# snf4j/snf4j

Measured on AMD Instinct MI355X. Metric: WebSocket frame decode GiB/s device-resident at 1/2/4/8 MI355X; % HBM peak, higher is better.
Workload: dtype u8; 1 GPU; 1048576 x 4096 B masked TEXT frames per GPU, 1024 sessions per GPU, unmask + UTF-8 validation, server-side decode (FrameDecoder+FrameUtf8Validator); frames_per_gpu=1048576, payload_bytes=4096, wire_bytes_per_gpu=4303355904, sessions_per_gpu=1024, parallelism=sessions sharded over 1 GPU(s), one process per GPU, no data-path collective

## Files before the change

snf4j_amd/build.py:

```python
from __future__ import annotations

import os
import subprocess
import sys
from concurrent.futures import ThreadPoolExecutor

HERE = os.path.dirname(os.path.abspath(__file__))
CSRC = os.path.join(HERE, "csrc")
OUT = os.path.join(HERE, "libwsgpu.so")
SOURCES = ["decode.hip", "encode.hip", "aggregate.hip", "api.hip", "batcher.hip", "inflate.hip", "handshake.hip", "deflate.hip"]
HEADERS = ["ws_rules.h", "wsgpu_internal.h", "wsgpu_scan.h", "deflate_core.h", "deflate_pmd.h", "../../include/wsgpu.h"]
BENCH_DIR = os.path.join(os.path.dirname(HERE), "benchsupport")
BENCH_SRC = os.path.join(BENCH_DIR, "csrc", "synth.hip")
BENCH_OUT = os.path.join(BENCH_DIR, "libwsbench.so")
BENCH_HDR = os.path.join(os.path.dirname(HERE), "include", "wsbench.h")
HIPCC = os.environ.get("HIPCC", "/opt/rocm/bin/hipcc")
FLAGS = ["--offload-arch=gfx950", "-O3", "-std=c++17", "-fPIC", "-Wall", "-Wno-unused-function",
         "-mllvm", "-disable-promote-alloca-to-lds"]


def _digest(paths, flags) -> str:
    import hashlib
    h = hashlib.sha256(" ".join(flags).encode())
    for p in paths:
        h.update(os.path.basename(p).encode())
        with open(p, "rb") as fh:
            h.update(fh.read())
    return h.hexdigest()


def _fresh(out: str, digest: str) -> bool:
    try:
        with open(out + ".srchash") as fh:
            return os.path.exists(out) and fh.read().strip() == digest
# ... 55 lines not shown
```

snf4j_amd/csrc/api.hip:

```cpp
#include <stdarg.h>
#include <stdio.h>
#include <stdlib.h>
#include <string.h>

#include <algorithm>
#include <atomic>
#include <string>
#include <vector>

#include "wsgpu_internal.h"

using namespace ws;

namespace {

std::atomic<uint64_t> g_ctx_allocs{0};

const char* const kKernelNames[K_COUNT] = {"k_parse",   "k_scan",     "k_link",     "k_piecesN",
                                           "k_final",    "k_enc_len",  "k_enc_scan",
                                           "k_enc_piecesN", "k_enc_final", "k_enc_desc", "k_agg_plan", "k_agg_gather", "k_inflate", "k_hs_accept", "k_infl_tok", "k_infl_fast", "k_hs_validate",
                                           "k_defl_plan", "k_defl_prep", "k_defl_match", "k_defl_parse", "k_defl_final", "k_defl_serial",
                                           "k_defl_trees", "k_defl_emit", "k_defl_hist", "k_defl_match_lds", "k_defl_links",
                                           "k_hs_accept_neg", "k_hs_validate_neg"};

// ... 295 lines not shown
}

int wsg_get_timing(wsg_ctx* c, double* out_ms, uint64_t* out_count, int max_kernels) {
  if (!c) return WSG_API_EINVAL;
  drain_timing(c);
  for (int i = 0; i < K_COUNT && i < max_kernels; ++i) {
    if (out_ms) out_ms[i] = c->ms[i];
    if (out_count) out_count[i] = c->count[i];
  }
  return K_COUNT;
}

int wsg_reset_timing(wsg_ctx* c) {
  if (!c) return WSG_API_EINVAL;
  drain_timing(c);
  memset(c->ms, 0, sizeof c->ms);
  memset(c->count, 0, sizeof c->count);
  return WSG_API_OK;
}

static int ensure_decode_ws(wsg_ctx* c, uint64_t n_frames, uint32_t n_sessions, uint64_t wire_len) {
  const uint64_t F = n_frames ? n_frames : 1;
  const uint64_t nblk = (F + DBLOCK - 1) / DBLOCK;
  HIP_TRY(c, c->pieces.ensure((piece_bound(wire_len, F) + 8) * sizeof(PieceDesc)));
  HIP_TRY(c, c->rec.ensure(F * sizeof(FrameRec)));
  HIP_TRY(c, c->vflag.ensure(F));
  HIP_TRY(c, c->slink.ensure(3 * (uint64_t)(n_sessions ? n_sessions : 1) * sizeof(int32_t)));
  HIP_TRY(c, c->edge.ensure(2 * F * sizeof(uint32_t)));
  HIP_TRY(c, c->blk_sum.ensure(nblk * sizeof(uint64_t)));
  HIP_TRY(c, c->blk_max.ensure(4 * ((nblk + 3) & ~3ull) * sizeof(int32_t)));
  HIP_TRY(c, c->chunk.ensure((nblk / SCAN_CHUNK + 1) * (sizeof(uint64_t) + 4 * sizeof(int32_t))));
  HIP_TRY(c, c->sess_err.ensure((uint64_t)(n_sessions ? n_sessions : 1) * sizeof(uint64_t), 0xff, c->stream));
  HIP_TRY(c, c->total.ensure(sizeof(uint64_t)));
  return WSG_API_OK;
}

static int ensure_encode_ws(wsg_ctx* c, uint64_t n_frames) {
  const uint64_t F = n_frames ? n_frames : 1;
  const uint64_t nblk = (F + BLOCK - 1) / BLOCK;
  HIP_TRY(c, c->esess.ensure(F * sizeof(uint32_t)));
  HIP_TRY(c, c->elast_close.ensure(F * sizeof(int32_t)));
  HIP_TRY(c, c->blk_sum.ensure(nblk * sizeof(uint64_t)));
  HIP_TRY(c, c->blk_max.ensure(3 * nblk * sizeof(int32_t)));
  return WSG_API_OK;
}

static constexpr uint64_t INFL_RESIDENT_LANES = 65536;
// ... 65 lines not shown
}
}

extern "C" {

int wsg_reserve(wsg_ctx* c, uint64_t max_frames, uint32_t max_sessions, uint64_t max_wire_len) {
  if (!c) return WSG_API_EINVAL;
  HIP_TRY(c, hipSetDevice(c->device));
  int rc = ensure_decode_ws(c, max_frames, max_sessions, max_wire_len);
  if (rc) return rc;
  return ensure_encode_ws(c, max_frames);
}

uint64_t wsg_decode_payload_bound(uint64_t wire_len, uint64_t n_frames) { return wire_len + 16 * n_frames + 16; }


int wsg_decode_batch_device(wsg_ctx* c, const wsg_decoder_cfg* cfg, const uint8_t* wire, uint64_t wire_len,
                            const uint64_t* frame_off, uint64_t n_frames, const uint32_t* session_first,
                            uint32_t n_sessions, wsg_session_state* state, uint8_t* payload_out,
                            uint64_t payload_cap, wsg_frame_desc* desc_out, wsg_session_result* result_out) {
  if (!c || !cfg) return WSG_API_EINVAL;
  if (n_sessions == 0) return n_frames ? set_err(c, WSG_API_EINVAL, "frames without sessions") : WSG_API_OK;
  if (n_frames >= (1ull << 30)) return set_err(c, WSG_API_ERANGE, "too many frames in one batch (max 2^30 - 1)");
  if (((uintptr_t)wire & 3) || ((uintptr_t)payload_out & 15))
    return set_err(c, WSG_API_EINVAL, "wire must be 4-B aligned and payload_out 16-B aligned");
  if (payload_cap < wire_len + 16 * n_frames)
    return set_err(c, WSG_API_ERANGE, "payload_cap below wsg_decode_payload_bound()");
  HIP_TRY(c, hipSetDevice(c->device));
  int rc = ensure_decode_ws(c, n_frames, n_sessions, wire_len);
  if (rc) return rc;
  DecodeArgs a;
  a.wire = wire;
  a.wire_len = wire_len;
  a.frame_off = frame_off;
  a.n_frames = n_frames;
  a.session_first = session_first;
  a.n_sessions = n_sessions;
  a.client_mode = cfg->client_mode != 0;
  a.allow_ext = cfg->allow_extensions != 0;
  a.validate = cfg->validate_utf8 != 0;
  a.max_payload = cfg->max_payload_len;
  a.state = state;
  a.payload_out = payload_out;
  a.desc = desc_out;
  a.result = result_out;
  a.rec = (FrameRec*)c->rec.p;
  a.vflag = (uint8_t*)c->vflag.p;
  a.slink = (int32_t*)c->slink.p;
  a.edge = (uint32_t*)c->edge.p;
  a.blk_sum = (uint64_t*)c->blk_sum.p;
  a.blk_max = (int32_t*)c->blk_max.p;
  a.chunk_sum = (uint64_t*)c->chunk.p;
  a.chunk_max = (int32_t*)(a.chunk_sum + (n_frames + DBLOCK - 1) / DBLOCK / SCAN_CHUNK + 1);
  a.sess_err = (uint64_t*)c->sess_err.p;
  a.total = (uint64_t*)c->total.p;
  a.pieces = (PieceDesc*)c->pieces.p;
  a.nblk = (uint32_t)((n_frames + DBLOCK - 1) / DBLOCK);
  a.n_pieces = piece_bound(wire_len, n_frames);
  a.validator_only = 0;
  a.in_desc = nullptr;
  a.sparse = (cfg->flags & WSG_CFG_SPARSE) != 0;
  a.fused_scan = a.nblk <= FUSED_SCAN_MAX_BLOCKS && c->fused_scan;
  if (n_frames) {
    timed(c, K_PARSE, [&] { launch_parse(a, c->stream); });
    if (!a.fused_scan) timed(c, K_SCAN, [&] { launch_scan(a, c->stream); });
    timed(c, K_LINK, [&] { launch_link(a, c->stream); });
    timed(c, K_UNMASK, [&] { launch_pieces(a, c->stream, piece_bound(wire_len, n_frames)); });
  }
  timed(c, K_FINAL, [&] { launch_final(a, c->stream); });
  HIP_TRY(c, hipGetLastError());
  return WSG_API_OK;
}

int wsg_validate_batch_device(wsg_ctx* c, const wsg_frame_desc* desc, uint64_t n_frames,
                              const uint32_t* session_first, uint32_t n_sessions, const uint8_t* payload,
                              uint64_t payload_len, wsg_session_state* state, wsg_session_result* result_out) {
  if (!c) return WSG_API_EINVAL;
  if (n_sessions == 0) return n_frames ? set_err(c, WSG_API_EINVAL, "frames without sessions") : WSG_API_OK;
  if (n_frames >= (1ull << 30)) return set_err(c, WSG_API_ERANGE, "too many frames in one batch (max 2^30 - 1)");
  if ((uintptr_t)payload & 3) return set_err(c, WSG_API_EINVAL, "payload must be 4-B aligned");
  HIP_TRY(c, hipSetDevice(c->device));
  int rc = ensure_decode_ws(c, n_frames, n_sessions, payload_len);
  if (rc) return rc;
  HIP_TRY(c, c->v_desc.ensure((n_frames + 1) * sizeof(wsg_frame_desc)));
  DecodeArgs a;
  a.wire = payload;
  a.wire_len = payload_len;
  a.frame_off = nullptr;
  a.n_frames = n_frames;
  a.session_first = session_first;
  a.n_sessions = n_sessions;
  a.client_mode = 0;
  a.allow_ext = 1;
  a.validate = 1;
  a.max_payload = INT64_MAX;
  a.state = state;
  a.payload_out = nullptr;
  a.desc = (wsg_frame_desc*)c->v_desc.p;
  a.result = result_out;
  a.rec = (FrameRec*)c->rec.p;
  a.vflag = (uint8_t*)c->vflag.p;
  a.slink = (int32_t*)c->slink.p;
  a.edge = (uint32_t*)c->edge.p;
  a.blk_sum = (uint64_t*)c->blk_sum.p;
  a.blk_max = (int32_t*)c->blk_max.p;
  a.chunk_sum = (uint64_t*)c->chunk.p;
  a.chunk_max = (int32_t*)(a.chunk_sum + (n_frames + DBLOCK - 1) / DBLOCK / SCAN_CHUNK + 1);
  a.sess_err = (uint64_t*)c->sess_err.p;
  a.total = (uint64_t*)c->total.p;
  a.pieces = (PieceDesc*)c->pieces.p;
  a.nblk = (uint32_t)((n_frames + DBLOCK - 1) / DBLOCK);
  a.n_pieces = piece_bound(payload_len, n_frames);
  a.validator_only = 1;
  a.in_desc = desc;
  a.sparse = 0;
  a.fused_scan = a.nblk <= FUSED_SCAN_MAX_BLOCKS && c->fused_scan;
  if (n_frames) {
    timed(c, K_PARSE, [&] { launch_vparse(a, c->stream); });
    if (!a.fused_scan) timed(c, K_SCAN, [&] { launch_scan(a, c->stream); });
    timed(c, K_LINK, [&] { launch_link(a, c->stream); });
    timed(c, K_UNMASK, [&] { launch_vpieces(a, c->stream, a.n_pieces); });
  }
  timed(c, K_FINAL, [&] { launch_final(a, c->stream); });
  HIP_TRY(c, hipGetLastError());
  return WSG_API_OK;
}

int wsg_validate_batch_host(wsg_ctx* c, const wsg_frame_desc* desc, uint64_t n_frames, const uint32_t* session_first,
                            uint32_t n_sessions, const uint8_t* payload, uint64_t payload_len, wsg_session_state* state,
                            wsg_session_result* result_out) {
  if (!c) return WSG_API_EINVAL;
  HIP_TRY(c, hipSetDevice(c->device));
  const uint64_t S = n_sessions;
  HIP_TRY(c, c->h_desc.ensure((n_frames + 1) * sizeof(wsg_frame_desc)));
  HIP_TRY(c, c->h_sf.ensure((S + 1) * sizeof(uint32_t)));
// ... 987 lines not shown
```

snf4j_amd/csrc/decode.hip:

```cpp
#include "wsgpu_internal.h"
#include "wsgpu_scan.h"

namespace ws {

__device__ bool utf8_valid_run(const uint8_t* wire, uint64_t off, uint32_t n, uint32_t mask, uint32_t phase0) {
  uint32_t p1 = 0, p2 = 0, p3 = 0;
  for (uint32_t i = 0; i < n; ++i) {
    uint32_t b = wire[off + i] ^ ((mask >> (8 * ((phase0 + i) & 3))) & 0xffu);
    if (utf8_err_byte(p3, p2, p1, b)) return false;
    p3 = p2; p2 = p1; p1 = b;
  }
  return !utf8_incomplete(p3, p2, p1);
}

struct DAgg {
  uint64_t sum;
  int32_t m0, m1, m2;
  uint32_t c3;
};
constexpr DAgg DAGG_ID = {0ull, -1, -1, -1, 0u};
constexpr uint32_t C3_RESET = 1u << 26;
constexpr uint32_t C3_PENDING = 1u << 27;

__device__ __forceinline__ uint32_t carry_op(uint32_t x, uint32_t y) {
// ... 321 lines not shown
    ex = agg_op(ex, e[i]);
  }
  if (threadIdx.x == 0) store_chunk(a, blockIdx.x, tot);
}

__device__ bool seam_utf8_error(uint32_t c3, uint32_t f3, uint32_t len, bool fin) {
  const uint32_t nc = (c3 >> 24) & 3u, nh = len < 3 ? len : 3u, n = nc + nh;
  const uint64_t win = (uint64_t)((c3 & 0xffffffu) >> (24 - 8 * nc)) | ((uint64_t)f3 << (8 * nc));
  for (uint32_t i = nc; i < n; ++i) {
    const uint32_t p1 = i >= 1 ? (uint32_t)(win >> (8 * (i - 1))) & 0xffu : 0u;
    const uint32_t p2 = i >= 2 ? (uint32_t)(win >> (8 * (i - 2))) & 0xffu : 0u;
    const uint32_t p3 = i >= 3 ? (uint32_t)(win >> (8 * (i - 3))) & 0xffu : 0u;
    if (utf8_err_byte(p3, p2, p1, (uint32_t)(win >> (8 * i)) & 0xffu)) return true;
  }
  if (fin && len < 3) {
    const uint32_t t1 = n >= 1 ? (uint32_t)(win >> (8 * (n - 1))) & 0xffu : 0u;
    const uint32_t t2 = n >= 2 ? (uint32_t)(win >> (8 * (n - 2))) & 0xffu : 0u;
    const uint32_t t3 = n >= 3 ? (uint32_t)(win >> (8 * (n - 3))) & 0xffu : 0u;
    if (utf8_incomplete(t3, t2, t1)) return true;
  }
  return false;
}

__device__ __forceinline__ void write_pieces(const DecodeArgs& a, bool live, uint64_t k, const FrameRec& r,
                                             uint64_t ex_sum, bool validate, bool cont, int lane) {
  const uint64_t slot = live ? (uint64_t)((r.len + 15u) & ~15u) : 0ull;
  const uint64_t slot_end = ex_sum + slot;
  const uint32_t pc0 = (uint32_t)((ex_sum + PIECE - 1) / PIECE);
  const uint32_t cnt = slot ? (uint32_t)((slot_end + PIECE - 1) / PIECE) - pc0 : 0u;
  uint32_t cum = cnt;
  cum = wave_incl_sum_u32(cum);
  const uint32_t T = (uint32_t)__builtin_amdgcn_readlane((int)cum, 63);
  cum -= cnt;
  if (!T) return;
  const uint32_t fk = (uint32_t)k | (validate ? 0x80000000u : 0u) | ((live && (r.code & CODE_FIN)) ? 0x40000000u : 0u);
  for (uint32_t t = lane; t < ((T + 63u) & ~63u); t += 64) {
    int o = 0;
#pragma unroll
    for (int step = 32; step >= 1; step >>= 1)
      if ((uint32_t)__shfl((int)cum, o + step, 64) <= t) o += step;
    const uint32_t o_cum = (uint32_t)__shfl((int)cum, o, 64);
    const uint32_t o_pc0 = (uint32_t)__shfl((int)pc0, o, 64);
    const uint64_t o_out = ((uint64_t)(uint32_t)__shfl((int)(uint32_t)(ex_sum >> 32), o, 64) << 32) |
                           (uint32_t)__shfl((int)(uint32_t)ex_sum, o, 64);
    const uint64_t o_src = ((uint64_t)(uint32_t)__shfl((int)(uint32_t)(r.src >> 32), o, 64) << 32) |
                           (uint32_t)__shfl((int)(uint32_t)r.src, o, 64);
    const uint32_t o_len = (uint32_t)__shfl((int)r.len, o, 64);
    const uint32_t o_mask = (uint32_t)__shfl((int)r.mask, o, 64);
    const uint32_t o_fk = (uint32_t)__shfl((int)fk, o, 64);
    const bool o_cont = __shfl((int)cont, o, 64) != 0;
    if (t >= T) continue;
    const uint64_t pc = (uint64_t)o_pc0 + (t - o_cum);
    if (pc >= a.n_pieces) continue;
    const uint64_t ps = pc * PIECE;
    const uint64_t o_end = o_out + ((o_len + 15u) & ~15u);
    const uint32_t j0 = (uint32_t)(ps - o_out);
    const uint32_t left = o_len - j0;
    const bool single = o_end >= ps + PIECE || (uint64_t)(o_fk & 0x3fffffffu) + 1 == a.n_frames;
    PieceDesc d;
    d.info = ((o_src + j0) & PD_SRC_MASK) | ((uint64_t)(left < PIECE ? left : PIECE) << PD_NB_SHIFT) |
             ((o_fk & 0x80000000u) ? PD_VALIDATE : 0ull) | (j0 == 0 ? PD_FIRST : 0ull) | (single ? 0ull : PD_MULTI) |
             (left <= PIECE ? PD_LAST : 0ull) | ((o_fk & 0x40000000u) ? PD_FIN : 0ull);
    d.mask = o_mask;
    d.frame = (o_fk & PDF_INDEX) | (o_cont ? PDF_CONT : 0u);
    a.pieces[pc] = d;
  }
}

__global__ __launch_bounds__(DBLOCK) void k_link(DecodeArgs a) {
  const int lane = threadIdx.x & 63;
  DAgg bp;
  if (a.fused_scan) {
    __shared__ uint32_t c3s[FUSED_SCAN_MAX_BLOCKS];
    DAgg t = DAGG_ID;
    const uint32_t nb = blockIdx.x, st = blk_stride(a);
    for (uint32_t b = threadIdx.x * 4u; b < nb; b += DBLOCK * 4u) {
      if (b + 4u <= nb) {
        const int4 x0 = *reinterpret_cast<const int4*>(a.blk_max + b);
        const int4 x1 = *reinterpret_cast<const int4*>(a.blk_max + st + b);
        const int4 x2 = *reinterpret_cast<const int4*>(a.blk_max + 2 * st + b);
        const int4 x3 = *reinterpret_cast<const int4*>(a.blk_max + 3 * st + b);
        const ulonglong2 s0 = *reinterpret_cast<const ulonglong2*>(a.blk_sum + b);
        const ulonglong2 s1 = *reinterpret_cast<const ulonglong2*>(a.blk_sum + b + 2);
        t.sum += s0.x + s0.y + s1.x + s1.y;
        t.m0 = max(max(t.m0, max(x0.x, x0.y)), max(x0.z, x0.w));
        t.m1 = max(max(t.m1, max(x1.x, x1.y)), max(x1.z, x1.w));
        t.m2 = max(max(t.m2, max(x2.x, x2.y)), max(x2.z, x2.w));
        c3s[b] = (uint32_t)x3.x;
// ... 59 lines not shown
        if (!a.validator_only) frag_err = rules_frag(op, frag);
        if (a.validate) {
          text = op == WSG_OP_TEXT;
          if (op == WSG_OP_CONTINUATION) text = jm >= sf ? (ex.m1 & 1) != 0 : (st.text_open != 0);
        }
      }
      uint32_t status = code_pre(r.code) ? code_pre(r.code) : (frag_err ? frag_err : code_post(r.code));
      if (!status && ex.sum + r.len > a.n_pieces * PIECE) status = WSG_E_BATCH;
      if (!status && text && op == WSG_OP_CONTINUATION &&
          seam_utf8_error(first ? tail_c3(st) : resolve_c3(ex.c3, st), a.edge[k], r.len, (r.code & CODE_FIN) != 0))
        status = WSG_E_TEXT_UTF8;
      validate = (text && !status) ? 1u : 0u;
      a.vflag[k] = (uint8_t)(validate | ((validate && op == WSG_OP_CONTINUATION) ? 2u : 0u));
      wsg_frame_desc d;
      d.payload_off = ex.sum;
      d.payload_len = r.len;
      d.opcode = (uint8_t)op;
      d.flags = (uint8_t)(((r.code & CODE_FIN) ? 0x80u : 0u) | (((r.code >> CODE_RSV_SHIFT) & 7u) << 4) |
                          ((r.code & CODE_MASKED) ? 1u : 0u));
      d.status = (uint16_t)status;
      a.desc[k] = d;
      if (status) atomicMin((unsigned long long*)&a.sess_err[s], (unsigned long long)k);
      if (k + 1 == a.session_first[s + 1]) {
        a.slink[s] = code_is_data(r.code) ? (int32_t)k : jd;
        a.slink[a.n_sessions + s] = code_is_start(r.code) ? (int32_t)k : jm;
        a.slink[2 * a.n_sessions + s] = (int32_t)resolve_c3(first ? v.c3 : carry_op(ex.c3, v.c3), st);
      }
    }
    write_pieces(a, live, k, r, ex.sum, validate != 0, live && code_op(r.code) == WSG_OP_CONTINUATION, lane);
  }
}

__global__ __launch_bounds__(DBLOCK) void k_vlink(DecodeArgs a) {
  const int lane = threadIdx.x & 63;
  VAgg bp;
  if (a.fused_scan) {
    __shared__ uint32_t fas[FUSED_SCAN_MAX_BLOCKS], fbs[FUSED_SCAN_MAX_BLOCKS];
    const uint32_t nb = blockIdx.x, st = blk_stride(a);
    uint64_t sum = 0;
    for (uint32_t b = threadIdx.x; b < nb; b += DBLOCK) {
      sum += a.blk_sum[b];
      fas[b] = (uint32_t)a.blk_max[b];
      fbs[b] = (uint32_t)a.blk_max[st + b];
    }
    __syncthreads();
    const uint32_t per = (nb + DBLOCK - 1) / DBLOCK;
    const uint32_t b0 = threadIdx.x * per, b1 = b0 + per < nb ? b0 + per : nb;
    VAgg t = VAGG_ID;
    for (uint32_t b = b0; b < b1; ++b) t = agg_op(t, VAgg{0ull, fas[b], fbs[b]});
    t.sum = sum;
    block_excl_scan_t(t, &bp, VAGG_ID);
  } else {
// ... 35 lines not shown
    if (ex.sum + r.len > a.n_pieces * PIECE) status = WSG_E_BATCH;
    if (!status && seam) {
      const uint32_t nh = r.len < 3 ? r.len : 3u;
      const uint32_t f3 = nh ? plain_word(a, r.src) & (0xffffffu >> (8 * (3 - nh))) : 0u;
      if (seam_utf8_error(carry, f3, r.len, (r.code & CODE_FIN) != 0)) status = WSG_E_TEXT_UTF8;
    }
    validate = validate && !status;
    seam = seam && validate;
    a.vflag[k] = (uint8_t)((validate ? 1u : 0u) | (seam ? 2u : 0u));
    wsg_frame_desc d;
    d.payload_off = ex.sum;
    d.payload_len = r.len;
    d.opcode = (uint8_t)op;
    d.flags = (uint8_t)(((r.code & CODE_FIN) ? 0x80u : 0u) | (((r.code >> CODE_RSV_SHIFT) & 7u) << 4));
    d.status = (uint16_t)status;
    a.desc[k] = d;
    if (status) atomicMin((unsigned long long*)&a.sess_err[s], (unsigned long long)k);
    if (k + 1 == a.session_first[s + 1]) {
      const VAgg inc = agg_op(ex, v);
      a.slink[a.n_sessions + s] = (int32_t)vopen(inc.fa);
      a.slink[2 * a.n_sessions + s] = (int32_t)inc.fb;
    }
  }
  write_pieces(a, live, k, r, ex.sum, validate, seam, lane);
}

__device__ __forceinline__ uint32_t dpp_from_next(uint32_t v, uint32_t old) {
  return (uint32_t)__builtin_amdgcn_update_dpp((int)old, (int)v, 0x130, 0xf, 0xf, false);
}
__device__ __forceinline__ uint32_t dpp_from_prev(uint32_t v, uint32_t old) {
  return (uint32_t)__builtin_amdgcn_update_dpp((int)old, (int)v, 0x138, 0xf, 0xf, false);
}

__device__ __forceinline__ uint32_t keep_bytes(uint32_t w, int keep) {
  return keep >= 4 ? w : (keep <= 0 ? 0u : (w & ((1u << (8 * keep)) - 1u)));
}
__device__ __forceinline__ uint32_t keep_flags(int keep) {
  return keep >= 4 ? 0x80808080u : (keep <= 0 ? 0u : (0x80808080u >> (8 * (4 - keep))));
}

__device__ __forceinline__ bool tail_error(uint32_t l3, bool fin) {
  return utf8_bad_last((l3 >> 16) & 0xffu) || (fin && utf8_incomplete(l3 & 0xffu, (l3 >> 8) & 0xffu, (l3 >> 16) & 0xffu));
}
__device__ __forceinline__ uint32_t last3(uint32_t pw, uint32_t w0, uint32_t w1, uint32_t w2, uint32_t w3, int keep) {
  const int t = keep + 1;
  const int q = t >> 2;
  const uint32_t lo = q == 0 ? pw : (q == 1 ? w0 : (q == 2 ? w1 : (q == 3 ? w2 : w3)));
  const uint32_t hi = q == 0 ? w0 : (q == 1 ? w1 : (q == 2 ? w2 : w3));
  return alignbyte(hi, lo, (uint32_t)t & 3u) & 0xffffffu;
}

__device__ __forceinline__ void report_utf8(const DecodeArgs& a, uint32_t k) {
  a.desc[k].status = (uint16_t)WSG_E_TEXT_UTF8;
  atomicMin((unsigned long long*)&a.sess_err[a.rec[k].sess], (unsigned long long)k);
}

__device__ __forceinline__ uint32_t prev_word(const DecodeArgs& a, uint64_t pos, uint32_t mask) {
  uint32_t w = 0;
  for (int i = 0; i < 4; ++i) w |= (uint32_t)a.wire[pos - 4 + i] << (8 * i);
  return w ^ mask;
}

template <int NT>
__device__ __forceinline__ uint32_t piece_fast(const DecodeArgs& a, const PieceDesc d, uint64_t pstart, int lane) {
  const uint32_t aux = (NT & 1) ? 2 : 0;
  constexpr bool ST = !(NT & 4);
  const uint64_t s = d.info & PD_SRC_MASK;
  const uint32_t nb = (uint32_t)(d.info >> PD_NB_SHIFT) & 2047u;
  const uint64_t a16 = s & ~15ull;
  const uint32_t sh = (uint32_t)(s & 15u);
  const uint32_t boff = (uint32_t)lane * 16u;
  const __amdgpu_buffer_rsrc_t rout =
      __builtin_amdgcn_make_buffer_rsrc((void*)(a.payload_out + pstart), 0, (int)PIECE, 0x00020000);
  const uint32_t b = sh & 3u;
  const uint64_t pva = a16 >= 16u ? a16 - 16u : 0u;
  const uint32_t i0 = 3u + (sh >> 2);
  const uint32_t pv_lo = ((const uint32_t*)(a.wire + pva))[i0];
  const uint32_t pv_hi = ((const uint32_t*)(a.wire + pva))[i0 + 1];
  u32x4 A;
  uint32_t e0, e1, e2, e3;
  if (a16 + PIECE + 16u <= a.wire_len) {
    const __amdgpu_buffer_rsrc_t rin =
        __builtin_amdgcn_make_buffer_rsrc((void*)(a.wire + a16), 0, (int)(PIECE + 16u), 0x00020000);
    A = __builtin_amdgcn_raw_buffer_load_b128(rin, boff, 0, aux);
    const u32x4 nx = *(const u32x4*)(a.wire + a16 + PIECE);
    e0 = nx.x; e1 = nx.y; e2 = nx.z; e3 = nx.w;
  } else {
    uint32_t dd[4] = {0u, 0u, 0u, 0u};
    for (uint32_t i = 0; i < 16u; ++i)
      if (a16 + boff + i < a.wire_len) dd[i >> 2] |= (uint32_t)a.wire[a16 + boff + i] << (8 * (i & 3));
    A = (u32x4){dd[0], dd[1], dd[2], dd[3]};
// ... 142 lines not shown
  if (pstart >= total) return;
  if (!(d.info & PD_MULTI)) {
    const uint32_t err = piece_fast<NT>(a, d, pstart, lane);
    if (__any(err != 0) && lane == 0) report_utf8(a, d.frame & PDF_INDEX);
    return;
  }
  piece_general<NT>(a, d, pstart, total, lane);
}

__device__ __forceinline__ void funnel16(uint32_t sh, uint32_t W0, uint32_t W1, uint32_t W2, uint32_t W3, uint32_t W4,
                                         uint32_t W5, uint32_t W6, uint32_t W7, uint32_t w[4]) {
  const uint32_t b = sh & 3u;
  switch (sh >> 2) {
    case 0: w[0] = alignbyte(W1, W0, b); w[1] = alignbyte(W2, W1, b); w[2] = alignbyte(W3, W2, b); w[3] = alignbyte(W4, W3, b); break;
    case 1: w[0] = alignbyte(W2, W1, b); w[1] = alignbyte(W3, W2, b); w[2] = alignbyte(W4, W3, b); w[3] = alignbyte(W5, W4, b); break;
    case 2: w[0] = alignbyte(W3, W2, b); w[1] = alignbyte(W4, W3, b); w[2] = alignbyte(W5, W4, b); w[3] = alignbyte(W6, W5, b); break;
    default: w[0] = alignbyte(W4, W3, b); w[1] = alignbyte(W5, W4, b); w[2] = alignbyte(W6, W5, b); w[3] = alignbyte(W7, W6, b); break;
  }
}

template <int NT, int N>
__device__ __forceinline__ uint32_t piece_fastN(const DecodeArgs& a, const PieceDesc d, const uint64_t info_last,
                                                uint64_t pstart, int lane) {
  const uint32_t nb_last = (uint32_t)(info_last >> PD_NB_SHIFT) & 2047u;
  const uint32_t aux = (NT & 1) ? 2 : 0;
  constexpr bool ST = !(NT & 4);
  const uint64_t s = d.info & PD_SRC_MASK;
  const uint64_t a16 = s & ~15ull;
  const uint32_t sh = (uint32_t)(s & 15u);
  const uint32_t boff = (uint32_t)lane * 16u;
  const __amdgpu_buffer_rsrc_t rout =
      __builtin_amdgcn_make_buffer_rsrc((void*)(a.payload_out + pstart), 0, (int)(N * PIECE), 0x00020000);
  const uint32_t b = sh & 3u;
  const uint64_t pva = a16 >= 16u ? a16 - 16u : 0u;
  const uint32_t i0 = 3u + (sh >> 2);
  const uint32_t pv_lo = ((const uint32_t*)(a.wire + pva))[i0];
  const uint32_t pv_hi = ((const uint32_t*)(a.wire + pva))[i0 + 1];
  u32x4 A[N];
  u32x4 nx;
  if (a16 + N * PIECE + 16u <= a.wire_len) {
    const __amdgpu_buffer_rsrc_t rin =
        __builtin_amdgcn_make_buffer_rsrc((void*)(a.wire + a16), 0, (int)(N * PIECE + 16u), 0x00020000);
#pragma unroll
    for (int i = 0; i < N; ++i) A[i] = __builtin_amdgcn_raw_buffer_load_b128(rin, boff + i * PIECE, 0, aux);
    nx = *(const u32x4*)(a.wire + a16 + N * PIECE);
  } else {
#pragma unroll
    for (int i = 0; i <= N; ++i) {
      uint32_t dd[4] = {0u, 0u, 0u, 0u};
      const uint64_t base = a16 + (uint64_t)i * PIECE + (i < N ? boff : 0u);
// ... 52 lines not shown
#pragma unroll
  for (int i = 0; i < N; ++i) {
    const uint32_t pw = dpp_from_prev(w[i][3], carry);
    U8W up, u0, u1, u2, u3;
    u8w_one(pw, up);
    u8w_pair(w[i][0], w[i][1], u0, u1);
    u8w_pair(w[i][2], w[i][3], u2, u3);
    uint32_t f0 = u8w_err(u0, up), f1 = u8w_err(u1, u0), f2 = u8w_err(u2, u1), f3 = u8w_err(u3, u2);
    const bool cont_head = i == 0 && lane == 0 && (d.info & PD_FIRST) && (d.frame & PDF_CONT);
    if (cont_head) f0 &= 0x80000000u;
    if (i + 1 == N && !full) {
      f0 &= keep_flags(keep); f1 &= keep_flags(keep - 4); f2 &= keep_flags(keep - 8); f3 &= keep_flags(keep - 12);
    }
    if (i + 1 == N && (info_last & PD_LAST) && keep >= 1 && keep <= 16) {
      const bool ge3 = N > 1 || !(lane == 0 && (d.info & PD_FIRST) && (d.frame & PDF_CONT) && keep < 3);
      if (tail_error(last3(pw, w[i][0], w[i][1], w[i][2], w[i][3], keep), ge3 && (info_last & PD_FIN))) err |= 1u;
    }
    err |= (f0 | f1 | f2 | f3) & H80;
    if (i + 1 < N) carry = (uint32_t)__builtin_amdgcn_readlane((int)w[i][3], 63);
  }
  return err;
}

template <int NT, int XCD, int N, int WPB = 1, int MINW = 1>
__global__ __launch_bounds__(64 * WPB) __attribute__((amdgpu_waves_per_eu(MINW))) void k_piecesN(DecodeArgs a) {
  const int lane = threadIdx.x & 63;
  const uint32_t blk = XCD ? xcd_remap(blockIdx.x, gridDim.x) : blockIdx.x;
  const uint64_t p = (uint64_t)N * (uint64_t)__builtin_amdgcn_readfirstlane(blk * (uint32_t)WPB + (threadIdx.x >> 6));
  if (WPB > 1 && p >= a.n_pieces) return;
  PieceDesc d[N];
#pragma unroll
  for (int i = 0; i < N; ++i) d[i] = a.pieces[p + i];
  const uint64_t total = *a.total;
  asm volatile("" ::"s"(d[0].info), "s"(d[0].mask), "s"(d[0].frame), "s"(d[N - 1].info), "s"(d[N - 1].frame),
               "s"(total));
  const uint64_t pstart = p * PIECE;
  if (pstart >= total) return;
  bool fast = pstart + (uint64_t)(N - 1) * PIECE < total && d[0].frame == d[N - 1].frame;
#pragma unroll
  for (int i = 0; i < N; ++i) fast = fast && !(d[i].info & PD_MULTI);
  if (fast) {
    const uint32_t err = piece_fastN<NT, N>(a, d[0], d[N - 1].info, pstart, lane);
    if (__any(err != 0) && lane == 0) report_utf8(a, d[0].frame & PDF_INDEX);
    return;
  }
#pragma unroll
  for (int i = 0; i < N; ++i) {
    const uint64_t ps = pstart + (uint64_t)i * PIECE;
    if (ps >= total) return;
    if (!(d[i].info & PD_MULTI)) {
      const uint32_t err = piece_fast<NT>(a, d[i], ps, lane);
      if (__any(err != 0) && lane == 0) report_utf8(a, d[i].frame & PDF_INDEX);
// ... 31 lines not shown
  const uint64_t fe = a.sess_err[s];
  if (fe != ~0ull) a.sess_err[s] = ~0ull;
  if (st.closed) {
    a.result[s] = res;
    return;
  }
  if (fe != ~0ull) {
    const uint32_t err = a.desc[fe].status;
    res.n_delivered = (uint32_t)(fe - sf);
    res.error = (uint16_t)err;
    res.close_code = close_code_of(err);
    res.detail = error_detail(a, fe, err);
    st.closed = 1;
  } else {
    res.n_delivered = se - sf;
    if (se > sf && a.validator_only) {
      const bool open = a.slink[a.n_sessions + s] != 0;
      const uint32_t c3 = (uint32_t)a.slink[2 * a.n_sessions + s];
      const uint32_t n = open ? (c3 >> 24) & 3u : 0u;
      for (uint32_t i = 0; i < n; ++i) st.tail[i] = (uint8_t)(c3 >> (24 - 8 * (n - i)));
      st.tail_len = (uint8_t)n;
      st.text_open = open;
    } else if (se > sf) {
      const int32_t ld = a.slink[s];
      if (ld >= (int32_t)sf) {
        const bool frag = !(a.rec[ld].code & CODE_FIN);
        st.fragmentation = frag;
        bool text = false;
        if (a.validate && frag) {
          const int32_t ls = a.slink[a.n_sessions + s];
          text = ls >= (int32_t)sf ? code_op(a.rec[ls].code) == WSG_OP_TEXT : (st.text_open != 0);
        }
        if (text) {
          const uint32_t c3 = (uint32_t)a.slink[2 * a.n_sessions + s];
          const uint32_t n = (c3 >> 24) & 3u;
          for (uint32_t i = 0; i < n; ++i) st.tail[i] = (uint8_t)(c3 >> (24 - 8 * (n - i)));
          st.tail_len = (uint8_t)n;
        } else {
          st.tail_len = 0;
        }
        st.text_open = text;
      }
    }
  }
  a.state[s] = st;
  a.result[s] = res;
}

void launch_parse(const DecodeArgs& a, hipStream_t s) {
  hipLaunchKernelGGL(k_parse, dim3(a.nblk), dim3(DBLOCK), 0, s, a);
}
void launch_scan(const DecodeArgs& a, hipStream_t s) {
  const dim3 g((a.nblk + SCAN_CHUNK - 1) / SCAN_CHUNK);
  if (a.validator_only) hipLaunchKernelGGL(k_scan<VAgg>, g, dim3(1024), 0, s, a);
  else hipLaunchKernelGGL(k_scan<DAgg>, g, dim3(1024), 0, s, a);
}
void launch_link(const DecodeArgs& a, hipStream_t s) {
  if (a.validator_only) hipLaunchKernelGGL(k_vlink, dim3(a.nblk), dim3(DBLOCK), 0, s, a);
  else hipLaunchKernelGGL(k_link, dim3(a.nblk), dim3(DBLOCK), 0, s, a);
}
#ifndef WSG_DWPB
#define WSG_DWPB 1
#endif
void launch_pieces(const DecodeArgs& a, hipStream_t s, uint64_t n_pieces_bound) {
  const uint64_t waves = (n_pieces_bound + PIECES_PER_WAVE - 1) / PIECES_PER_WAVE;
  hipLaunchKernelGGL((k_piecesN<1, 1, PIECES_PER_WAVE, WSG_DWPB>), dim3((uint32_t)((waves + WSG_DWPB - 1) / WSG_DWPB)),
                     dim3(64 * WSG_DWPB), 0, s, a);
}
void launch_vparse(const DecodeArgs& a, hipStream_t s) {
  hipLaunchKernelGGL(k_vparse, dim3(a.nblk), dim3(DBLOCK), 0, s, a);
}
#ifndef WSG_VWPB
#define WSG_VWPB 1
#endif
#ifndef WSG_VMINW
#define WSG_VMINW 1
#endif
void launch_vpieces(const DecodeArgs& a, hipStream_t s, uint64_t n_pieces_bound) {
  const uint64_t waves = (n_pieces_bound + VPIECES_PER_WAVE - 1) / VPIECES_PER_WAVE;
  hipLaunchKernelGGL((k_piecesN<5, 1, VPIECES_PER_WAVE, WSG_VWPB, WSG_VMINW>), dim3((uint32_t)((waves + WSG_VWPB - 1) / WSG_VWPB)),
                     dim3(64 * WSG_VWPB), 0, s, a);
}
void launch_final(const DecodeArgs& a, hipStream_t s) {
  hipLaunchKernelGGL(k_final, dim3((a.n_sessions + 255) / 256), dim3(256), 0, s, a);
}

}
```

snf4j_amd/csrc/wsgpu_internal.h:

```cpp
#pragma once
#include <stdint.h>

#include <hip/hip_runtime.h>

#include "ws_rules.h"

namespace ws {

struct FrameRec {
  uint64_t src;
  uint32_t len;
  uint32_t mask;
  uint32_t code;
  uint32_t sess;
};

constexpr uint32_t CODE_PRE_SHIFT = 0;
constexpr uint32_t CODE_POST_SHIFT = 5;
constexpr uint32_t CODE_FRAG_SHIFT = 10;
constexpr uint32_t CODE_FIN = 1u << 16;
constexpr uint32_t CODE_RSV_SHIFT = 17;
constexpr uint32_t CODE_MASKED = 1u << 20;
constexpr uint32_t CODE_OP_SHIFT = 24;

__host__ __device__ inline uint32_t code_pre(uint32_t c) { return (c >> CODE_PRE_SHIFT) & 31u; }
__host__ __device__ inline uint32_t code_post(uint32_t c) { return (c >> CODE_POST_SHIFT) & 31u; }
__host__ __device__ inline uint32_t code_frag(uint32_t c) { return (c >> CODE_FRAG_SHIFT) & 31u; }
__host__ __device__ inline uint32_t code_op(uint32_t c) { return (c >> CODE_OP_SHIFT) & 15u; }
// ... 5 lines not shown
constexpr int BLOCK = 256;
#ifndef WSG_AGG_BLOCK
#define WSG_AGG_BLOCK 512
#endif
constexpr int ABLOCK = WSG_AGG_BLOCK;
#ifndef WSG_DBLOCK
#define WSG_DBLOCK 256
#endif
constexpr int DBLOCK = WSG_DBLOCK;
constexpr uint32_t PIECE = 1024;
constexpr int PIECES_PER_WAVE = 2;
#ifndef WSG_VPIECES
#define WSG_VPIECES 4
#endif
constexpr int VPIECES_PER_WAVE = WSG_VPIECES;
#ifndef WSG_ENC_PIECES
#define WSG_ENC_PIECES 2
#endif
constexpr int ENC_PIECES_PER_WAVE = WSG_ENC_PIECES;

__host__ __device__ inline uint64_t piece_bound(uint64_t wire_len, uint64_t n_frames) {
  return (wire_len + 16 * n_frames) / PIECE + 1;
}

struct PieceDesc {
  uint64_t info;
  uint32_t mask;
  uint32_t frame;
};
constexpr uint32_t PDF_INDEX = 0x3fffffffu;
constexpr uint32_t PDF_CONT = 0x80000000u;
constexpr uint64_t PD_SRC_MASK = (1ull << 48) - 1;
constexpr uint32_t PD_NB_SHIFT = 48;
constexpr uint64_t PD_VALIDATE = 1ull << 59;
constexpr uint64_t PD_FIRST = 1ull << 60;
constexpr uint64_t PD_MULTI = 1ull << 61;
constexpr uint64_t PD_LAST = 1ull << 62;
constexpr uint64_t PD_FIN = 1ull << 63;

struct DecodeArgs {
  const uint8_t* wire;
  uint64_t wire_len;
  const uint64_t* frame_off;
  uint64_t n_frames;
  const uint32_t* session_first;
  uint32_t n_sessions;
  int32_t client_mode, allow_ext, validate;
  int64_t max_payload;
  int32_t validator_only;
  const wsg_frame_desc* in_desc;
  int32_t sparse;
  wsg_session_state* state;
  uint8_t* payload_out;
  wsg_frame_desc* desc;
  wsg_session_result* result;
  FrameRec* rec;
  uint8_t* vflag;
  int32_t* slink;
  uint32_t* edge;
  uint64_t* blk_sum;
  int32_t* blk_max;
  uint64_t* chunk_sum;
  int32_t* chunk_max;
  uint64_t* sess_err;
  uint64_t* total;
  struct PieceDesc* pieces;
  uint64_t n_pieces;
  uint32_t nblk;
  int32_t fused_scan;
};

constexpr uint32_t FUSED_SCAN_MAX_BLOCKS = 4096;
constexpr uint32_t SCAN_CHUNK = 4096;

struct EncodeArgs {
  int32_t client_mode;
  const uint8_t* payload;
  uint64_t payload_len;
  const wsg_encode_frame* frames;
  uint64_t n_frames;
  const uint32_t* session_first;
  uint32_t n_sessions;
  uint8_t* closed;
  uint8_t* wire_out;
  uint64_t wire_cap;
  uint64_t* wire_off;
  uint32_t* sess;
  uint64_t* blk_sum;
  int32_t* blk_max;
// ... 261 lines not shown
```

Before: 2819 GiB/s.

## Describe decode work in two-piece units with a side array for odd pieces

The piece descriptor table for the decode path becomes one descriptor per unit of two 1 KiB pieces, plus a separate array for odd-piece descriptors that is used only where a frame boundary splits a unit. A unit that lies entirely inside one frame is flagged simple, so a wave reads one descriptor and runs the fast two-piece path. The aim is to cut descriptor writes and reads and the scalar work per wave. It also packs session-link metadata into the slink values so the final kernel no longer re-reads FrameRec, and it narrows the source field to 47 bits, adding new wire_len limits.

```diff
diff --git a/snf4j_amd/build.py b/snf4j_amd/build.py
--- a/snf4j_amd/build.py
+++ b/snf4j_amd/build.py
@@ -9,7 +9,7 @@
 CSRC = os.path.join(HERE, "csrc")
 OUT = os.path.join(HERE, "libwsgpu.so")
 SOURCES = ["decode.hip", "encode.hip", "aggregate.hip", "api.hip", "batcher.hip", "inflate.hip", "handshake.hip", "deflate.hip"]
-HEADERS = ["ws_rules.h", "wsgpu_internal.h", "wsgpu_scan.h", "deflate_core.h", "deflate_pmd.h", "../../include/wsgpu.h"]
+HEADERS = ["ws_rules.h", "wsgpu_internal.h", "wsgpu_units.h", "wsgpu_scan.h", "deflate_core.h", "deflate_pmd.h", "../../include/wsgpu.h"]
 BENCH_DIR = os.path.join(os.path.dirname(HERE), "benchsupport")
 BENCH_SRC = os.path.join(BENCH_DIR, "csrc", "synth.hip")
 BENCH_OUT = os.path.join(BENCH_DIR, "libwsbench.so")
diff --git a/snf4j_amd/csrc/api.hip b/snf4j_amd/csrc/api.hip
--- a/snf4j_amd/csrc/api.hip
+++ b/snf4j_amd/csrc/api.hip
@@ -341,7 +341,7 @@
 static int ensure_decode_ws(wsg_ctx* c, uint64_t n_frames, uint32_t n_sessions, uint64_t wire_len) {
   const uint64_t F = n_frames ? n_frames : 1;
   const uint64_t nblk = (F + DBLOCK - 1) / DBLOCK;
-  HIP_TRY(c, c->pieces.ensure((piece_bound(wire_len, F) + 8) * sizeof(PieceDesc)));
+  HIP_TRY(c, c->pieces.ensure((2 * decode_units(piece_bound(wire_len, F)) + 8) * sizeof(PieceDesc)));
   HIP_TRY(c, c->rec.ensure(F * sizeof(FrameRec)));
   HIP_TRY(c, c->vflag.ensure(F));
   HIP_TRY(c, c->slink.ensure(3 * (uint64_t)(n_sessions ? n_sessions : 1) * sizeof(int32_t)));
@@ -453,6 +453,7 @@
   if (!c || !cfg) return WSG_API_EINVAL;
   if (n_sessions == 0) return n_frames ? set_err(c, WSG_API_EINVAL, "frames without sessions") : WSG_API_OK;
   if (n_frames >= (1ull << 30)) return set_err(c, WSG_API_ERANGE, "too many frames in one batch (max 2^30 - 1)");
+  if (wire_len > UD_SRC_MASK) return set_err(c, WSG_API_ERANGE, "wire_len must be below 2^47");
   if (((uintptr_t)wire & 3) || ((uintptr_t)payload_out & 15))
     return set_err(c, WSG_API_EINVAL, "wire must be 4-B aligned and payload_out 16-B aligned");
   if (payload_cap < wire_len + 16 * n_frames)
@@ -488,6 +489,7 @@
   a.pieces = (PieceDesc*)c->pieces.p;
   a.nblk = (uint32_t)((n_frames + DBLOCK - 1) / DBLOCK);
   a.n_pieces = piece_bound(wire_len, n_frames);
+  a.odd = a.pieces + decode_units(a.n_pieces);
   a.validator_only = 0;
   a.in_desc = nullptr;
   a.sparse = (cfg->flags & WSG_CFG_SPARSE) != 0;
@@ -509,6 +511,7 @@
   if (!c) return WSG_API_EINVAL;
   if (n_sessions == 0) return n_frames ? set_err(c, WSG_API_EINVAL, "frames without sessions") : WSG_API_OK;
   if (n_frames >= (1ull << 30)) return set_err(c, WSG_API_ERANGE, "too many frames in one batch (max 2^30 - 1)");
+  if (payload_len > UD_SRC_MASK) return set_err(c, WSG_API_ERANGE, "payload_len must be below 2^47");
   if ((uintptr_t)payload & 3) return set_err(c, WSG_API_EINVAL, "payload must be 4-B aligned");
   HIP_TRY(c, hipSetDevice(c->device));
   int rc = ensure_decode_ws(c, n_frames, n_sessions, payload_len);
@@ -542,6 +545,7 @@
   a.pieces = (PieceDesc*)c->pieces.p;
   a.nblk = (uint32_t)((n_frames + DBLOCK - 1) / DBLOCK);
   a.n_pieces = piece_bound(payload_len, n_frames);
+  a.odd = nullptr;
   a.validator_only = 1;
   a.in_desc = desc;
   a.sparse = 0;
diff --git a/snf4j_amd/csrc/decode.hip b/snf4j_amd/csrc/decode.hip
--- a/snf4j_amd/csrc/decode.hip
+++ b/snf4j_amd/csrc/decode.hip
@@ -367,12 +367,14 @@
   return false;
 }
 
+template <bool UNITS>
 __device__ __forceinline__ void write_pieces(const DecodeArgs& a, bool live, uint64_t k, const FrameRec& r,
                                              uint64_t ex_sum, bool validate, bool cont, int lane) {
   const uint64_t slot = live ? (uint64_t)((r.len + 15u) & ~15u) : 0ull;
   const uint64_t slot_end = ex_sum + slot;
-  const uint32_t pc0 = (uint32_t)((ex_sum + PIECE - 1) / PIECE);
-  const uint32_t cnt = slot ? (uint32_t)((slot_end + PIECE - 1) / PIECE) - pc0 : 0u;
+  uint32_t cnt;
+  if (UNITS) cnt = slot_desc_count(slot_units(ex_sum, slot, k + 1 == a.n_frames));
+  else cnt = slot ? (uint32_t)((slot_end + PIECE - 1) / PIECE) - (uint32_t)((ex_sum + PIECE - 1) / PIECE) : 0u;
   uint32_t cum = cnt;
   cum = wave_incl_sum_u32(cum);
   const uint32_t T = (uint32_t)__builtin_amdgcn_readlane((int)cum, 63);
@@ -385,7 +387,6 @@
     for (int step = 32; step >= 1; step >>= 1)
       if ((uint32_t)__shfl((int)cum, o + step, 64) <= t) o += step;
     const uint32_t o_cum = (uint32_t)__shfl((int)cum, o, 64);
-    const uint32_t o_pc0 = (uint32_t)__shfl((int)pc0, o, 64);
     const uint64_t o_out = ((uint64_t)(uint32_t)__shfl((int)(uint32_t)(ex_sum >> 32), o, 64) << 32) |
                            (uint32_t)__shfl((int)(uint32_t)ex_sum, o, 64);
     const uint64_t o_src = ((uint64_t)(uint32_t)__shfl((int)(uint32_t)(r.src >> 32), o, 64) << 32) |
@@ -395,20 +396,34 @@
     const uint32_t o_fk = (uint32_t)__shfl((int)fk, o, 64);
     const bool o_cont = __shfl((int)cont, o, 64) != 0;
     if (t >= T) continue;
-    const uint64_t pc = (uint64_t)o_pc0 + (t - o_cum);
+    const uint64_t o_slot = (uint64_t)((o_len + 15u) & ~15u);
+    const bool o_last = (uint64_t)(o_fk & 0x3fffffffu) + 1 == a.n_frames;
+    uint64_t pc;
+    bool odd = false, simple = false;
+    if (UNITS) {
+      const SlotItem it = slot_item(slot_units(o_out, o_slot, o_last), t - o_cum, o_out, o_slot, o_last);
+      pc = it.piece;
+      odd = it.odd != 0;
+      simple = it.simple && pc + 1 < a.n_pieces;
+    } else {
+      pc = (o_out + PIECE - 1) / PIECE + (t - o_cum);
+    }
     if (pc >= a.n_pieces) continue;
     const uint64_t ps = pc * PIECE;
-    const uint64_t o_end = o_out + ((o_len + 15u) & ~15u);
+    const uint64_t o_end = o_out + o_slot;
     const uint32_t j0 = (uint32_t)(ps - o_out);
     const uint32_t left = o_len - j0;
-    const bool single = o_end >= ps + PIECE || (uint64_t)(o_fk & 0x3fffffffu) + 1 == a.n_frames;
+    const uint32_t span = simple ? PIECES_PER_WAVE * PIECE : PIECE;
+    const bool single = simple || o_end >= ps + PIECE || o_last;
     PieceDesc d;
-    d.info = ((o_src + j0) & PD_SRC_MASK) | ((uint64_t)(left < PIECE ? left : PIECE) << PD_NB_SHIFT) |
+    d.info = ((o_src + j0) & UD_SRC_MASK) | ((uint64_t)(left < span ? left : span) << UD_NB_SHIFT) |
              ((o_fk & 0x80000000u) ? PD_VALIDATE : 0ull) | (j0 == 0 ? PD_FIRST : 0ull) | (single ? 0ull : PD_MULTI) |
-             (left <= PIECE ? PD_LAST : 0ull) | ((o_fk & 0x40000000u) ? PD_FIN : 0ull);
+             (left <= span ? PD_LAST : 0ull) | ((o_fk & 0x40000000u) ? PD_FIN : 0ull);
     d.mask = o_mask;
-    d.frame = (o_fk & PDF_INDEX) | (o_cont ? PDF_CONT : 0u);
-    a.pieces[pc] = d;
+    d.frame = (o_fk & PDF_INDEX) | (o_cont ? PDF_CONT : 0u) | (simple ? PDF_SIMPLE : 0u);
+    if (!UNITS) a.pieces[pc] = d;
+    else if (odd) a.odd[pc >> 1] = d;
+    else a.pieces[pc >> 1] = d;
   }
 }
 
@@ -514,12 +529,12 @@
       a.desc[k] = d;
       if (status) atomicMin((unsigned long long*)&a.sess_err[s], (unsigned long long)k);
       if (k + 1 == a.session_first[s + 1]) {
-        a.slink[s] = code_is_data(r.code) ? (int32_t)k : jd;
-        a.slink[a.n_sessions + s] = code_is_start(r.code) ? (int32_t)k : jm;
+        a.slink[s] = code_is_data(r.code) ? v.m0 : ex.m0;
+        a.slink[a.n_sessions + s] = code_is_start(r.code) ? v.m1 : ex.m1;
         a.slink[2 * a.n_sessions + s] = (int32_t)resolve_c3(first ? v.c3 : carry_op(ex.c3, v.c3), st);
       }
     }
-    write_pieces(a, live, k, r, ex.sum, validate != 0, live && code_op(r.code) == WSG_OP_CONTINUATION, lane);
+    write_pieces<true>(a, live, k, r, ex.sum, validate != 0, live && code_op(r.code) == WSG_OP_CONTINUATION, lane);
   }
 }
 
@@ -601,7 +616,7 @@
       a.slink[2 * a.n_sessions + s] = (int32_t)inc.fb;
     }
   }
-  write_pieces(a, live, k, r, ex.sum, validate, seam, lane);
+  write_pieces<false>(a, live, k, r, ex.sum, validate, seam, lane);
 }
 
 __device__ __forceinline__ uint32_t dpp_from_next(uint32_t v, uint32_t old) {
@@ -644,8 +659,8 @@
 __device__ __forceinline__ uint32_t piece_fast(const DecodeArgs& a, const PieceDesc d, uint64_t pstart, int lane) {
   const uint32_t aux = (NT & 1) ? 2 : 0;
   constexpr bool ST = !(NT & 4);
-  const uint64_t s = d.info & PD_SRC_MASK;
-  const uint32_t nb = (uint32_t)(d.info >> PD_NB_SHIFT) & 2047u;
+  const uint64_t s = d.info & UD_SRC_MASK;
+  const uint32_t nb = (uint32_t)(d.info >> UD_NB_SHIFT) & UD_NB_MASK;
   const uint64_t a16 = s & ~15ull;
   const uint32_t sh = (uint32_t)(s & 15u);
   const uint32_t boff = (uint32_t)lane * 16u;
@@ -834,10 +849,10 @@
 template <int NT, int N>
 __device__ __forceinline__ uint32_t piece_fastN(const DecodeArgs& a, const PieceDesc d, const uint64_t info_last,
                                                 uint64_t pstart, int lane) {
-  const uint32_t nb_last = (uint32_t)(info_last >> PD_NB_SHIFT) & 2047u;
+  const uint32_t nb_last = (uint32_t)(info_last >> UD_NB_SHIFT) & UD_NB_MASK;
   const uint32_t aux = (NT & 1) ? 2 : 0;
   constexpr bool ST = !(NT & 4);
-  const uint64_t s = d.info & PD_SRC_MASK;
+  const uint64_t s = d.info & UD_SRC_MASK;
   const uint64_t a16 = s & ~15ull;
   const uint32_t sh = (uint32_t)(s & 15u);
   const uint32_t boff = (uint32_t)lane * 16u;
@@ -936,12 +951,64 @@
   return err;
 }
 
-template <int NT, int XCD, int N, int WPB = 1, int MINW = 1>
+__device__ __forceinline__ PieceDesc load_desc_const(const PieceDesc* p) {
+  typedef __attribute__((address_space(4))) const uint64_t* const_u64;
+  const const_u64 q = (const_u64)(uintptr_t)p;
+  const uint64_t info = q[0], mf = q[1];
+  return PieceDesc{info, (uint32_t)mf, (uint32_t)(mf >> 32)};
+}
+
+#ifndef WSG_HOIST_KERNARGS
+#define WSG_HOIST_KERNARGS 1
+#endif
+
+template <int NT, int XCD, int N, int WPB = 1, int MINW = 1, bool UNITS = false>
 __global__ __launch_bounds__(64 * WPB) __attribute__((amdgpu_waves_per_eu(MINW))) void k_piecesN(DecodeArgs a) {
   const int lane = threadIdx.x & 63;
   const uint32_t blk = XCD ? xcd_remap(blockIdx.x, gridDim.x) : blockIdx.x;
   const uint64_t p = (uint64_t)N * (uint64_t)__builtin_amdgcn_readfirstlane(blk * (uint32_t)WPB + (threadIdx.x >> 6));
   if (WPB > 1 && p >= a.n_pieces) return;
+  if (UNITS) {
+    static_assert(!UNITS || N == PIECES_PER_WAVE, "a unit is PIECES_PER_WAVE pieces");
+    const PieceDesc u = a.pieces[p / N];
+    uint64_t total = *a.total;
+#if WSG_HOIST_KERNARGS
+    asm("" : "+s"(total) : "s"(u.info), "s"(u.mask), "s"(u.frame), "s"(a.wire), "s"(a.wire_len), "s"(a.payload_out),
+        "s"(a.desc), "s"(a.rec), "s"(a.vflag));
+#else
+    asm("" : "+s"(total) : "s"(u.info), "s"(u.mask), "s"(u.frame));
+#endif
+    const uint64_t pstart = p * PIECE;
+    if (pstart >= total) return;
+    if (u.frame & PDF_SIMPLE) {
+      const uint32_t nb = (uint32_t)(u.info >> UD_NB_SHIFT) & UD_NB_MASK;
+      uint32_t err;
+      if (nb > PIECE) {
+        const uint64_t info_last = (u.info & ~((uint64_t)UD_NB_MASK << UD_NB_SHIFT)) | ((uint64_t)(nb - PIECE) << UD_NB_SHIFT);
+        err = piece_fastN<NT, N>(a, u, info_last, pstart, lane);
+      } else {
+        err = piece_fast<NT>(a, u, pstart, lane);
+      }
+      if (__any(err != 0) && lane == 0) report_utf8(a, u.frame & PDF_INDEX);
+      return;
+    }
+    const bool has_odd = __builtin_amdgcn_readfirstlane((int)(pstart + PIECE < total && p + 1 < a.n_pieces)) != 0;
+    PieceDesc o = {0ull, 0u, 0u};
+    if (has_odd) o = load_desc_const(a.odd + p / N);
+#pragma unroll
+    for (int i = 0; i < N; ++i) {
+      const uint64_t ps = pstart + (uint64_t)i * PIECE;
+      if (i && !has_odd) return;
+      const PieceDesc d = i ? o : u;
+      if (!(d.info & PD_MULTI)) {
+        const uint32_t err = piece_fast<NT>(a, d, ps, lane);
+        if (__any(err != 0) && lane == 0) report_utf8(a, d.frame & PDF_INDEX);
+      } else {
+        piece_general<NT>(a, d, ps, total, lane);
+      }
+    }
+    return;
+  }
   PieceDesc d[N];
 #pragma unroll
   for (int i = 0; i < N; ++i) d[i] = a.pieces[p + i];
@@ -1019,14 +1086,14 @@
       st.tail_len = (uint8_t)n;
       st.text_open = open;
     } else if (se > sf) {
-      const int32_t ld = a.slink[s];
-      if (ld >= (int32_t)sf) {
-        const bool frag = !(a.rec[ld].code & CODE_FIN);
+      const int32_t m0 = a.slink[s];
+      if ((m0 >> 1) >= (int32_t)sf) {
+        const bool frag = !(m0 & 1);
         st.fragmentation = frag;
         bool text = false;
         if (a.validate && frag) {
-          const int32_t ls = a.slink[a.n_sessions + s];
-          text = ls >= (int32_t)sf ? code_op(a.rec[ls].code) == WSG_OP_TEXT : (st.text_open != 0);
+          const int32_t m1 = a.slink[a.n_sessions + s];
+          text = (m1 >> 1) >= (int32_t)sf ? (m1 & 1) != 0 : (st.text_open != 0);
         }
         if (text) {
           const uint32_t c3 = (uint32_t)a.slink[2 * a.n_sessions + s];
@@ -1061,8 +1128,8 @@
 #endif
 void launch_pieces(const DecodeArgs& a, hipStream_t s, uint64_t n_pieces_bound) {
   const uint64_t waves = (n_pieces_bound + PIECES_PER_WAVE - 1) / PIECES_PER_WAVE;
-  hipLaunchKernelGGL((k_piecesN<1, 1, PIECES_PER_WAVE, WSG_DWPB>), dim3((uint32_t)((waves + WSG_DWPB - 1) / WSG_DWPB)),
-                     dim3(64 * WSG_DWPB), 0, s, a);
+  hipLaunchKernelGGL((k_piecesN<1, 1, PIECES_PER_WAVE, WSG_DWPB, 1, true>),
+                     dim3((uint32_t)((waves + WSG_DWPB - 1) / WSG_DWPB)), dim3(64 * WSG_DWPB), 0, s, a);
 }
 void launch_vparse(const DecodeArgs& a, hipStream_t s) {
   hipLaunchKernelGGL(k_vparse, dim3(a.nblk), dim3(DBLOCK), 0, s, a);
diff --git a/snf4j_amd/csrc/wsgpu_internal.h b/snf4j_amd/csrc/wsgpu_internal.h
--- a/snf4j_amd/csrc/wsgpu_internal.h
+++ b/snf4j_amd/csrc/wsgpu_internal.h
@@ -4,6 +4,7 @@
 #include <hip/hip_runtime.h>
 
 #include "ws_rules.h"
+#include "wsgpu_units.h"
 
 namespace ws {
 
@@ -55,6 +56,9 @@
 __host__ __device__ inline uint64_t piece_bound(uint64_t wire_len, uint64_t n_frames) {
   return (wire_len + 16 * n_frames) / PIECE + 1;
 }
+__host__ __device__ inline uint64_t decode_units(uint64_t n_pieces) {
+  return (n_pieces + PIECES_PER_WAVE - 1) / PIECES_PER_WAVE;
+}
 
 struct PieceDesc {
   uint64_t info;
@@ -70,6 +74,11 @@
 constexpr uint64_t PD_MULTI = 1ull << 61;
 constexpr uint64_t PD_LAST = 1ull << 62;
 constexpr uint64_t PD_FIN = 1ull << 63;
+
+constexpr uint64_t UD_SRC_MASK = (1ull << 47) - 1;
+constexpr uint32_t UD_NB_SHIFT = 47;
+constexpr uint32_t UD_NB_MASK = 4095u;
+constexpr uint32_t PDF_SIMPLE = 0x40000000u;
 
 struct DecodeArgs {
   const uint8_t* wire;
@@ -98,6 +107,7 @@
   uint64_t* sess_err;
   uint64_t* total;
   struct PieceDesc* pieces;
+  struct PieceDesc* odd;
   uint64_t n_pieces;
   uint32_t nblk;
   int32_t fused_scan;
diff --git a/snf4j_amd/csrc/wsgpu_units.h b/snf4j_amd/csrc/wsgpu_units.h
--- /dev/null
+++ b/snf4j_amd/csrc/wsgpu_units.h
@@ -0,0 +1,59 @@
+#pragma once
+#include <stdint.h>
+
+#include "ws_rules.h"
+
+namespace ws {
+
+constexpr uint64_t UNIT_PIECE = 1024;
+constexpr uint64_t UNIT_BYTES = 2 * UNIT_PIECE;
+
+struct SlotUnits {
+  uint32_t u0;
+  uint32_t nu;
+  uint32_t lead;
+  uint32_t trail;
+};
+
+WS_HD SlotUnits slot_units(uint64_t o, uint64_t slot, bool last) {
+  SlotUnits r;
+  const uint64_t e = o + slot;
+  const uint64_t u0 = (o + UNIT_BYTES - 1) / UNIT_BYTES, u1 = (e + UNIT_BYTES - 1) / UNIT_BYTES;
+  r.u0 = (uint32_t)u0;
+  r.nu = slot ? (uint32_t)(u1 - u0) : 0u;
+  const uint64_t h = u0 * UNIT_BYTES - UNIT_PIECE;
+  r.lead = (slot && u0 && h >= o && h < e) ? 1u : 0u;
+  r.trail = (r.nu && !last && e < u1 * UNIT_BYTES && e > u1 * UNIT_BYTES - UNIT_PIECE) ? 1u : 0u;
+  return r;
+}
+
+WS_HD uint32_t slot_desc_count(const SlotUnits& s) { return s.lead + s.nu + s.trail; }
+
+struct SlotItem {
+  uint32_t piece;
+  uint32_t odd;
+  uint32_t simple;
+};
+
+WS_HD SlotItem slot_item(const SlotUnits& s, uint32_t t, uint64_t o, uint64_t slot, bool last) {
+  SlotItem it;
+  it.simple = 0u;
+  if (t < s.lead) {
+    it.piece = 2u * s.u0 - 1u;
+    it.odd = 1u;
+    return it;
+  }
+  t -= s.lead;
+  if (t < s.nu) {
+    const uint64_t u = (uint64_t)s.u0 + t;
+    it.piece = (uint32_t)(2u * u);
+    it.odd = 0u;
+    it.simple = (last || o + slot >= (u + 1) * UNIT_BYTES) ? 1u : 0u;
+    return it;
+  }
+  it.piece = 2u * (s.u0 + s.nu) - 1u;
+  it.odd = 1u;
+  return it;
+}
+
+}
```

Result: no change. 2840 GiB/s, median of 6 (+0.7%).
